# SSTDV-Project/python-fluid-simulation

Measured on AMD Instinct MI355X. Metric: PressureCGSolver3D CG throughput (cells x iterations / s), higher is better.
Workload: dtype f32; 1 GPU; PressureCGSolver3D 256x256x256 synthetic pool scene, fp32 state; cells_per_gpu=16777216, decomposition=single domain, transport=single, step=one CG iteration (apply + 2 dots + x/r/d updates)

## Files before the change

python-fluid-simulation_amd/csrc/mfs_pcg_apply.h:

```cpp
#pragma once
#include "mfs_common.h"
#include "mfs_cg_core.h"

#define MFS_LDS_BARRIER() asm volatile("s_waitcnt lgkmcnt(0)\n\ts_barrier" ::: "memory")

#ifndef MFS_MARCH_MIN_WAVES
#define MFS_MARCH_MIN_WAVES 3
#endif

namespace mfs {

constexpr int kApplyBlock = 256;
constexpr int kXcds = 8;

template <typename T, int VEC>
__device__ __forceinline__ void stencil_vec(T* __restrict__ out_ptr, vec_t<T, VEC> vc, vec_t<T, VEC> vxp,
                                            vec_t<T, VEC> vxm, vec_t<T, VEC> vyp, vec_t<T, VEC> vym,
                                            vec_t<T, VEC> dg, vec_t<T, VEC> cxp, vec_t<T, VEC> cxm,
                                            vec_t<T, VEC> cyp, vec_t<T, VEC> cym, vec_t<T, VEC> czm, double zl,
                                            double zr, double czr, bool first, bool last, bool active, double& acc,
                                            vec_t<T, VEC> czm2) {
  vec_t<T, VEC> o;
#ifdef MFS_APPLY_NATIVE_MATH
  typedef T C;
#else
  typedef double C;
#endif
#pragma unroll
  for (int j = 0; j < VEC; ++j) {
    const C zm = j == 0 ? (C)zl : (C)vc[j == 0 ? 0 : j - 1];
    const C zp = j == VEC - 1 ? (C)zr : (C)vc[j == VEC - 1 ? j : j + 1];
    const C czp = j == VEC - 1 ? (C)czr : (C)czm[j == VEC - 1 ? j : j + 1];
    C val = 0;
    val -= (C)cxp[j] * (C)vxp[j];
    val -= (C)cxm[j] * (C)vxm[j];
    val -= (C)cyp[j] * (C)vyp[j];
    val -= (C)cym[j] * (C)vym[j];
    val -= czp * zp;
    val -= (C)czm2[j] * zm;
    val += (C)dg[j] * (C)vc[j];
    o[j] = (T)val;
    const bool bnd = (first && j == 0) || (last && j == VEC - 1);
    if (active && !bnd) acc += (double)vc[j] * (double)o[j];
  }
  if (!active) return;
  if (!first && !last) {
    vstore<T, VEC>(out_ptr, o);
  } else {
#pragma unroll
    for (int j = 0; j < VEC; ++j) {
      const bool bnd = (first && j == 0) || (last && j == VEC - 1);
      if (!bnd) out_ptr[j] = o[j];
    }
  }
}

struct ApplyArgs {
  int Nx, Ny, Nz, xb, xe, xchunk, xb2, xe2;
  const int* items = nullptr;
  const int* runrem = nullptr;
  const int* count = nullptr;
};

template <typename T, int VEC>
__global__ void __launch_bounds__(kApplyBlock)
k_pcg_apply_direct(const T* __restrict__ v, T* __restrict__ out, const T* __restrict__ diag,
                   const T* __restrict__ cx, const T* __restrict__ cy, const T* __restrict__ cz, ApplyArgs a,
                   double* __restrict__ partial, const double* __restrict__ done_flag) {
  if (done_flag && *done_flag != 0.0) return;
  const int nzv = a.Nz / VEC;
  const int64_t ipp = (int64_t)(a.Ny - 2) * nzv;
  const int n1 = a.xe - a.xb;
  const int np = n1 + (a.xe2 - a.xb2);
  const int nch = min((int)gridDim.x, kXcds);
  const int xcd = blockIdx.x % nch, slot = blockIdx.x / nch;
  const int nblk = (gridDim.x - xcd + nch - 1) / nch;
  const int p0 = (int)((int64_t)np * xcd / nch), p1 = (int)((int64_t)np * (xcd + 1) / nch);
  const int64_t end = (int64_t)p1 * ipp, stride = (int64_t)nblk * kApplyBlock;
  const int64_t sx = (int64_t)a.Ny * a.Nz, sy = a.Nz;
  double acc = 0.0;
  for (int64_t it = (int64_t)p0 * ipp + (int64_t)slot * kApplyBlock + threadIdx.x; it < end; it += stride) {
    const int px = (int)(it / ipp);
    const int rem = (int)(it - (int64_t)px * ipp);
    const int yy = rem / nzv, zv = rem - (rem / nzv) * nzv;
    const int xx = px < n1 ? a.xb + px : a.xb2 + (px - n1);
    const int64_t base = (int64_t)xx * sx + (int64_t)(yy + 1) * sy + (int64_t)zv * VEC;
    const bool first = zv == 0, last = zv == nzv - 1;
    const auto vc = vload<T, VEC>(v + base);
    const double zl = first ? 0.0 : (double)v[base - 1];
    const double zr = last ? 0.0 : (double)v[base + VEC];
    const double czr = last ? 0.0 : (double)cz[base + VEC];
    stencil_vec<T, VEC>(out + base, vc, vload<T, VEC>(v + base + sx), vload<T, VEC>(v + base - sx),
                        vload<T, VEC>(v + base + sy), vload<T, VEC>(v + base - sy), vload<T, VEC>(diag + base),
                        vload<T, VEC>(cx + base + sx), vload<T, VEC>(cx + base), vload<T, VEC>(cy + base + sy),
                        vload<T, VEC>(cy + base), vload<T, VEC>(cz + base), zl, zr, czr, first, last, true, acc,
                        vload<T, VEC>(cz + base));
  }
  const double tot = block_sum<kApplyBlock>(acc);
  if (threadIdx.x == 0) partial[blockIdx.x] = tot;
}


template <typename T, int VEC>
struct CoefVec {
  vec_t<T, VEC> dg, cxm, cxp, cym, cyp, czm, czm2;
  unsigned char cls;
};

template <typename T, int VEC, bool COMP, int NT, bool LOAD_CXM = true, bool ASYM = false>
__device__ __forceinline__ CoefVec<T, VEC> coef_load(const T* __restrict__ diag, const T* __restrict__ cx,
                                                     const T* __restrict__ cy, const T* __restrict__ cz,
                                                     int64_t b, int64_t sx, int Nz, unsigned char cls,
                                                     const T* __restrict__ cz2 = nullptr) {
  CoefVec<T, VEC> c;
  c.cls = cls;
  if (COMP) {
    const T f = cls == kClsRegular ? (T)1 : (T)0, d = cls == kClsRegular ? (T)6 : (T)0;
#pragma unroll
    for (int j = 0; j < VEC; ++j) { c.dg[j] = d; c.cxm[j] = f; c.cxp[j] = f; c.cym[j] = f; c.cyp[j] = f; c.czm[j] = f; c.czm2[j] = f; }
    if (cls == kClsMixed) {
      c.dg = (NT & 1) ? vload_nt<T, VEC>(diag + b) : vload<T, VEC>(diag + b);
      if (LOAD_CXM) c.cxm = vload<T, VEC>(cx + b);
      c.cxp = (NT & 2) ? vload_nt<T, VEC>(cx + b + sx) : vload<T, VEC>(cx + b + sx);
      c.cym = (NT & 4) ? vload_nt<T, VEC>(cy + b) : vload<T, VEC>(cy + b);
      c.cyp = (NT & 4) ? vload_nt<T, VEC>(cy + b + Nz) : vload<T, VEC>(cy + b + Nz);
      c.czm = (NT & 1) ? vload_nt<T, VEC>(cz + b) : vload<T, VEC>(cz + b);
      if (ASYM) c.czm2 = (NT & 1) ? vload_nt<T, VEC>(cz2 + b) : vload<T, VEC>(cz2 + b);
    }
    if (!ASYM) c.czm2 = c.czm;
    return c;
  }
  c.dg = (NT & 1) ? vload_nt<T, VEC>(diag + b) : vload<T, VEC>(diag + b);
  c.cxm = c.dg;
  c.cxp = (NT & 2) ? vload_nt<T, VEC>(cx + b + sx) : vload<T, VEC>(cx + b + sx);
  c.cym = (NT & 4) ? vload_nt<T, VEC>(cy + b) : vload<T, VEC>(cy + b);
  c.cyp = (NT & 4) ? vload_nt<T, VEC>(cy + b + Nz) : vload<T, VEC>(cy + b + Nz);
  c.czm = (NT & 1) ? vload_nt<T, VEC>(cz + b) : vload<T, VEC>(cz + b);
  if (ASYM) c.czm2 = (NT & 1) ? vload_nt<T, VEC>(cz2 + b) : vload<T, VEC>(cz2 + b);
  else c.czm2 = c.czm;
  return c;
}

template <typename T, int VEC>
__global__ void __launch_bounds__(256)
k_pcg_classify(const T* __restrict__ diag, const T* __restrict__ cx, const T* __restrict__ cy,
               const T* __restrict__ cz, int Nx, int Ny, int Nz, unsigned char* __restrict__ cls,
               const T* __restrict__ cz2) {
  const int nzv = Nz / VEC;
  const int64_t nvec = (int64_t)Nx * Ny * nzv;
  const int64_t iv = (int64_t)blockIdx.x * blockDim.x + threadIdx.x;
  if (iv >= nvec) return;
  const int zv = (int)(iv % nzv), y = (int)((iv / nzv) % Ny), x = (int)(iv / ((int64_t)nzv * Ny));
  const int64_t sx = (int64_t)Ny * Nz, b = iv * VEC;
  bool all_zero = true, all_reg = true;
  if (x > 0 && x < Nx - 1 && y > 0 && y < Ny - 1) {
#pragma unroll
    for (int j = 0; j < VEC; ++j) {
      const int z = zv * VEC + j;
      if (z == 0 || z == Nz - 1) continue;
      const int64_t c = b + j;
      const T k[7] = {diag[c], cx[c], cx[c + sx], cy[c], cy[c + Nz], cz2 ? cz2[c] : cz[c], cz[c + 1]};
      bool z0 = true, r1 = k[0] == (T)6;
#pragma unroll
      for (int q = 0; q < 7; ++q) { z0 = z0 && k[q] == (T)0; if (q) r1 = r1 && k[q] == (T)1; }
      if (cz2 && j == 0) { z0 = z0 && cz[c] == (T)0; r1 = r1 && cz[c] == (T)1; }
      all_zero = all_zero && z0;
      all_reg = all_reg && r1;
    }
  }
  cls[iv] = all_zero ? kClsZero : (all_reg ? kClsRegular : kClsMixed);
}

template <typename T, int VEC>
struct RawVec { vec_t<T, VEC> a, b; };

template <typename T, int VEC, bool FUSE>
struct VSrc {
  const T* __restrict__ v;
  const T* __restrict__ r;
  const T* __restrict__ d_old;
  double beta;
  __device__ __forceinline__ RawVec<T, VEC> raw(int64_t off) const {
    RawVec<T, VEC> w;
    if (!FUSE) { w.a = vload<T, VEC>(v + off); w.b = w.a; }
    else { w.a = vload<T, VEC>(r + off); w.b = vload<T, VEC>(d_old + off); }
    return w;
  }
  __device__ __forceinline__ vec_t<T, VEC> fin(const RawVec<T, VEC>& w) const {
    if (!FUSE) return w.a;
    vec_t<T, VEC> o;
#pragma unroll
    for (int j = 0; j < VEC; ++j) o[j] = (T)((double)w.a[j] + beta * (double)w.b[j]);
    return o;
  }
  __device__ __forceinline__ vec_t<T, VEC> ld(int64_t off) const { return fin(raw(off)); }
};

struct BookArgs {
  double* scal;
  double* hist;
  int64_t hist_cap;
  const double* part_rr;
  int npart, par;
};

template <typename T, int VEC, bool LDS, int NT, bool COMP, bool FUSE, int PD, bool ASYM = false, bool XDEF = false,
          bool BOOK = false, bool LMASK = false>
__global__ void __launch_bounds__(kApplyBlock, MFS_MARCH_MIN_WAVES)
k_pcg_apply_march(const T* __restrict__ v, T* __restrict__ out, const T* __restrict__ diag,
                  const T* __restrict__ cx, const T* __restrict__ cy, const T* __restrict__ cz,
                  const unsigned char* __restrict__ cls, ApplyArgs a, double* __restrict__ partial,
                  const double* __restrict__ done_flag, const T* __restrict__ fr, const T* __restrict__ fd_old,
                  T* __restrict__ fd_new, const double* __restrict__ beta_ptr, const T* __restrict__ cz2,
                  T* __restrict__ xdef = nullptr, const double* __restrict__ alpha_ptr = nullptr, BookArgs bk = BookArgs{}) {
  static_assert(!XDEF || FUSE, "the deferred x update rides on the fused direction update");
  static_assert(!LMASK || (COMP && FUSE && PD == 1), "lane-level masking: compressed, fused, prefetch depth 1");
  static_assert(!BOOK || FUSE, "closing the previous iteration rides on the fused direction update");
  static_assert(kApplyBlock == kBlock, "block_total_of is written for kBlock threads");
  double alpha_x = (XDEF && !BOOK) ? *alpha_ptr : 0.0;
  static_assert(!FUSE || LDS, "the fused direction update is implemented on the LDS march");
  double bk_dn = 0.0, bk_delta = 0.0, bk_dq = 0.0, bk_tol2 = 0.0, bk_acc = 0.0;
  bool book_pending = BOOK;
  double beta_v = 0.0;
  if (BOOK) {
    bk_dn = bk.scal[S_DONE]; bk_delta = bk.scal[S_RING + bk.par]; bk_dq = bk.scal[S_DQ]; bk_tol2 = bk.scal[S_TOL2];
    for (int i = threadIdx.x; i < bk.npart; i += kBlock) bk_acc += bk.part_rr[i];
  } else {
    if (done_flag && *done_flag != 0.0) return;
    if (FUSE) beta_v = *beta_ptr;
  }
  VSrc<T, VEC, FUSE> src{v, fr, fd_old, beta_v};
  extern __shared__ __align__(16) unsigned char smem_raw[];
  T* const smem = reinterpret_cast<T*>(smem_raw);
  const int Nz = a.Nz;
  const int nzv = Nz / VEC;
  const int ipp = (a.Ny - 2) * nzv;
  const int tiles = (ipp + kApplyBlock - 1) / kApplyBlock;
  const int n1 = a.xe - a.xb;
  const int np = n1 + (a.xe2 - a.xb2);
  const bool sparse = a.items != nullptr;
  const int64_t total = sparse ? (int64_t)*a.count : (int64_t)tiles * np;

  const int G = gridDim.x;
  const int nch = min(G, kXcds);
  const int xcd = blockIdx.x % nch, slot = blockIdx.x / nch;
  const int per = G / nch, extra = G - per * nch;
  const int seg = xcd * per + min(xcd, extra) + slot;
  const int64_t s0 = total * seg / G, s1 = total * (seg + 1) / G;
  const int64_t sx = (int64_t)a.Ny * Nz;
  const int tid = threadIdx.x, lane = tid & 63;
  const int tile_elems = kApplyBlock * VEC;
  const int buf_elems = tile_elems + 2 * Nz;
  double acc = 0.0;

  auto close_previous = [&]() -> bool {
    book_pending = false;
    __shared__ double s_rr;
    const double t = block_sum<kBlock>(bk_acc);
    if (threadIdx.x == 0) s_rr = t;
    __syncthreads();
    const double rr = s_rr;
    const bool stop = bk_dn != 0.0 || cg_health(bk_dq, rr) != 0 || rr < bk_tol2;
    if (bk_dn == 0.0 && blockIdx.x == 0 && threadIdx.x == 0) cg_book(bk.scal, bk.hist, bk.hist_cap, bk.par, bk_dq, rr);
    src.beta = rr / bk_delta;
    if (XDEF) alpha_x = bk_delta / bk_dq;
    return stop;
  };

  for (int64_t i = s0; i < s1;) {
    const int64_t it_ = sparse ? (int64_t)a.items[i] : i;
    const int tile = (int)(it_ / np);
    const int pl = (int)(it_ - (int64_t)tile * np);
    const int x0 = pl < n1 ? a.xb + pl : a.xb2 + (pl - n1);
    int len = (int)min((int64_t)((pl < n1 ? a.xe : a.xe2) - x0), s1 - i);
    if (sparse) len = min(len, a.runrem[i]);
    if (a.xchunk > 0) len = min(len, a.xchunk);
    const int x1 = x0 + len;
    i += len;
    const int item_raw = tile * kApplyBlock + tid;
    const bool active = item_raw < ipp;
    const int item = active ? item_raw : ipp - 1;
    const int yy = item / nzv, zv = item - yy * nzv;
    const bool first = zv == 0, last = zv == nzv - 1;
    const int64_t m = (int64_t)(yy + 1) * Nz + (int64_t)zv * VEC;
    const int64_t m0 = (int64_t)Nz + (int64_t)tile * tile_elems;
    const int tile_len = min(tile_elems, ipp * VEC - tile * tile_elems);

    int64_t base = (int64_t)x0 * sx + m;
    const RawVec<T, VEC> wm = src.raw(base - sx), wc = src.raw(base), wp = src.raw(base + sx);
    constexpr bool MASK = LMASK;
    const bool mask_on = MASK && sparse;
    unsigned char cls_n = kClsMixed, cls_c = kClsMixed, cls_n2 = kClsMixed;
    if (COMP) {
      cls_c = cls[base / VEC];
      cls_n = cls[(base + (x0 + 1 < x1 ? sx : 0)) / VEC];
      if (MASK) cls_n2 = cls[((int64_t)min(x0 + 2, x1) * sx + m) / VEC];
    }
    RawVec<T, VEC> wh = {};
    const bool h0 = LDS && tid < 2 * nzv;
    if (h0) wh = src.raw((int64_t)x0 * sx + (tid < nzv ? m0 - Nz + tid * VEC : m0 + tile_len + (tid - nzv) * VEC));
    if (BOOK && book_pending) {
      if (close_previous()) return;
    }
    vec_t<T, VEC> vm = src.fin(wm), vc = src.fin(wc), vp = src.fin(wp);
    CoefVec<T, VEC> cc = coef_load<T, VEC, COMP, NT, true, ASYM>(diag, cx, cy, cz, base, sx, Nz, cls_c, cz2);
    if (!COMP) cc.cxm = vload<T, VEC>(cx + base);

    if (LDS) {
      T* b0 = smem;
      if (active) vstore<T, VEC>(b0 + Nz + tid * VEC, vc);
      if (h0) vstore<T, VEC>(b0 + (tid < nzv ? tid * VEC : Nz + tile_len + (tid - nzv) * VEC), src.fin(wh));
      for (int s = tid + kApplyBlock; s < 2 * nzv; s += kApplyBlock) {
        const bool lo = s < nzv;
        const int j = lo ? s : s - nzv;
        vstore<T, VEC>(b0 + (lo ? j * VEC : Nz + tile_len + j * VEC),
                       src.ld((int64_t)x0 * sx + (lo ? m0 - Nz + j * VEC : m0 + tile_len + j * VEC)));
      }
      MFS_LDS_BARRIER();
    }
    const bool hact = LDS && tid < 2 * nzv;
    const bool hlow = tid < nzv;
    const int64_t hg = hlow ? m0 - Nz + (int64_t)tid * VEC : m0 + tile_len + (int64_t)(tid - nzv) * VEC;
    const int hl = hlow ? tid * VEC : Nz + tile_len + (tid - nzv) * VEC;
    RawVec<T, VEC> Q[PD > 1 ? PD - 1 : 1], H[PD];
#pragma unroll
    for (int k = 0; k < PD - 1; ++k) Q[k] = src.raw((int64_t)min(x0 + 2 + k, x1) * sx + m);
#pragma unroll
    for (int k = 0; k < PD; ++k) {
      H[k] = RawVec<T, VEC>{};
      if (hact) H[k] = src.raw((int64_t)min(x0 + 1 + k, x1) * sx + hg);
    }

    for (int x = x0; x < x1; ++x) {
      const bool more = x + 1 < x1;
      const int cur = (x - x0) & 1;
      const int64_t nb = base + sx;
      const int64_t nn = more ? nb : base;
      const int64_t n2 = more ? nb + sx : nb;
      const bool dead_c = mask_on && cc.cls == kClsDead;
      RawVec<T, VEC> qn = {};
      if (!(mask_on && cls_n2 == kClsDead)) qn = src.raw((int64_t)min(x + 1 + PD, x1) * sx + m);
      vec_t<T, VEC> xo = {}, dxo = {};
      if (XDEF && !dead_c) { xo = vload_nt<T, VEC>(xdef + base); dxo = vload<T, VEC>(fd_old + base); }
      CoefVec<T, VEC> cn = coef_load<T, VEC, COMP, NT, false, ASYM>(diag, cx, cy, cz, nn, sx, Nz, more ? cls_n : cc.cls, cz2);
      cn.cxm = cc.cxp;
      unsigned char cls_nn = kClsMixed;
      if (COMP) cls_nn = MASK ? cls[((int64_t)min(x + 3, x1) * sx + m) / VEC] : cls[n2 / VEC];
      RawVec<T, VEC> hn = {};
      if (hact) hn = src.raw((int64_t)min(x + 1 + PD, x1) * sx + hg);
      vec_t<T, VEC> vym, vyp;
      double zl, zr;
      if (LDS) {
        const T* bc = smem + cur * buf_elems;
        vym = vload<T, VEC>(bc + tid * VEC);
        vyp = vload<T, VEC>(bc + 2 * Nz + tid * VEC);
        zl = (double)bc[Nz + tid * VEC - 1];
        zr = (double)bc[Nz + tid * VEC + VEC];
      } else {
        vym = vload<T, VEC>(v + base - Nz);
        vyp = vload<T, VEC>(v + base + Nz);
        const T l = __shfl_up(vc[VEC - 1], 1, 64), r = __shfl_down(vc[0], 1, 64);
        zl = (double)((lane == 0 && !first) ? v[base - 1] : l);
        zr = (double)((lane == 63 && !last) ? v[base + VEC] : r);
      }
      const T czs = __shfl_down(cc.czm[0], 1, 64);
      const double czr = (double)((lane == 63 && !last) ? cz[base + VEC] : czs);
      stencil_vec<T, VEC>(out + base, vc, vp, vm, vyp, vym, cc.dg, cc.cxp, cc.cxm, cc.cyp, cc.cym, cc.czm, zl, zr, czr,
                          first, last, active && !dead_c, acc, cc.czm2);
      if (FUSE && active && !dead_c) vstore<T, VEC>(fd_new + base, vc);
      if (XDEF && active && !dead_c) {
#pragma unroll
        for (int j = 0; j < VEC; ++j) xo[j] = (T)((double)xo[j] + alpha_x * (double)dxo[j]);
        vstore_nt<T, VEC>(xdef + base, xo);
      }
      if (more) {
        if (LDS) {
          T* bn = smem + (cur ^ 1) * buf_elems;
          if (active) vstore<T, VEC>(bn + Nz + tid * VEC, vp);
          if (hact) vstore<T, VEC>(bn + hl, src.fin(H[0]));
          for (int s = tid + kApplyBlock; s < 2 * nzv; s += kApplyBlock) {
            const bool lo = s < nzv;
            const int j = lo ? s : s - nzv;
            vstore<T, VEC>(bn + (lo ? j * VEC : Nz + tile_len + j * VEC),
                           src.ld((int64_t)(x + 1) * sx + (lo ? m0 - Nz + j * VEC : m0 + tile_len + j * VEC)));
          }
          MFS_LDS_BARRIER();
        }
        vm = vc; vc = vp; vp = src.fin(PD == 1 ? qn : Q[0]); cc = cn;
        if (MASK) { cls_n = cls_n2; cls_n2 = cls_nn; } else cls_n = cls_nn;
#pragma unroll
        for (int k = 0; k + 1 < PD - 1; ++k) Q[k] = Q[k + 1];
        if (PD > 1) Q[PD - 2] = qn;
#pragma unroll
        for (int k = 0; k + 1 < PD; ++k) H[k] = H[k + 1];
        H[PD - 1] = hn;
        base = nb;
      }
    }
    if (LDS) MFS_LDS_BARRIER();
  }
  if (BOOK && book_pending) {
    if (close_previous()) return;
  }
  const double tot = block_sum<kApplyBlock>(acc);
  if (threadIdx.x == 0) partial[blockIdx.x] = tot;
}

}
```

Baseline: 191,900 Mcells/s.

## Reuse streamed direction values for deferred x update and reorder marching loads/stores

The deferred x += alpha*d_old update now takes d_old from the raw direction value already streamed for the stencil (the .b half of the fused source), so the separate fd_old reload is gone. The x loads are prefetched two planes ahead to match the stencil's read-ahead. The stencil is split into compute and store, and empty asm register constraints force the next plane's loads to be waited on before the output stores are issued. The z-edge coefficient is also prefetched one plane ahead. This cuts global reads and reorders the memory queue, but raises register pressure and restricts the deferred-x path to prefetch depth 1.

Result: faster. 194,700 Mcells/s (median of 6 runs) (+1.4%).

```diff
diff --git a/python-fluid-simulation_amd/csrc/mfs_pcg_apply.h b/python-fluid-simulation_amd/csrc/mfs_pcg_apply.h
--- a/python-fluid-simulation_amd/csrc/mfs_pcg_apply.h
+++ b/python-fluid-simulation_amd/csrc/mfs_pcg_apply.h
@@ -14,12 +14,12 @@
 constexpr int kXcds = 8;
 
 template <typename T, int VEC>
-__device__ __forceinline__ void stencil_vec(T* __restrict__ out_ptr, vec_t<T, VEC> vc, vec_t<T, VEC> vxp,
-                                            vec_t<T, VEC> vxm, vec_t<T, VEC> vyp, vec_t<T, VEC> vym,
-                                            vec_t<T, VEC> dg, vec_t<T, VEC> cxp, vec_t<T, VEC> cxm,
-                                            vec_t<T, VEC> cyp, vec_t<T, VEC> cym, vec_t<T, VEC> czm, double zl,
-                                            double zr, double czr, bool first, bool last, bool active, double& acc,
-                                            vec_t<T, VEC> czm2) {
+__device__ __forceinline__ vec_t<T, VEC> stencil_calc(vec_t<T, VEC> vc, vec_t<T, VEC> vxp,
+                                                      vec_t<T, VEC> vxm, vec_t<T, VEC> vyp, vec_t<T, VEC> vym,
+                                                      vec_t<T, VEC> dg, vec_t<T, VEC> cxp, vec_t<T, VEC> cxm,
+                                                      vec_t<T, VEC> cyp, vec_t<T, VEC> cym, vec_t<T, VEC> czm, double zl,
+                                                      double zr, double czr, bool first, bool last, bool active, double& acc,
+                                                      vec_t<T, VEC> czm2) {
   vec_t<T, VEC> o;
 #ifdef MFS_APPLY_NATIVE_MATH
   typedef T C;
@@ -43,6 +43,11 @@
     const bool bnd = (first && j == 0) || (last && j == VEC - 1);
     if (active && !bnd) acc += (double)vc[j] * (double)o[j];
   }
+  return o;
+}
+
+template <typename T, int VEC>
+__device__ __forceinline__ void stencil_put(T* __restrict__ out_ptr, vec_t<T, VEC> o, bool first, bool last, bool active) {
   if (!active) return;
   if (!first && !last) {
     vstore<T, VEC>(out_ptr, o);
@@ -54,6 +59,20 @@
     }
   }
 }
+
+template <typename T, int VEC>
+__device__ __forceinline__ void stencil_vec(T* __restrict__ out_ptr, vec_t<T, VEC> vc, vec_t<T, VEC> vxp,
+                                            vec_t<T, VEC> vxm, vec_t<T, VEC> vyp, vec_t<T, VEC> vym,
+                                            vec_t<T, VEC> dg, vec_t<T, VEC> cxp, vec_t<T, VEC> cxm,
+                                            vec_t<T, VEC> cyp, vec_t<T, VEC> cym, vec_t<T, VEC> czm, double zl,
+                                            double zr, double czr, bool first, bool last, bool active, double& acc,
+                                            vec_t<T, VEC> czm2) {
+  stencil_put<T, VEC>(out_ptr, stencil_calc<T, VEC>(vc, vxp, vxm, vyp, vym, dg, cxp, cxm, cyp, cym, czm, zl, zr, czr, first,
+                                                    last, active, acc, czm2), first, last, active);
+}
+
+template <typename S>
+__device__ __forceinline__ void vm_arrived(S s) { asm volatile("" ::"v"(s)); }
 
 struct ApplyArgs {
   int Nx, Ny, Nz, xb, xe, xchunk, xb2, xe2;
@@ -213,7 +232,7 @@
                   const double* __restrict__ done_flag, const T* __restrict__ fr, const T* __restrict__ fd_old,
                   T* __restrict__ fd_new, const double* __restrict__ beta_ptr, const T* __restrict__ cz2,
                   T* __restrict__ xdef = nullptr, const double* __restrict__ alpha_ptr = nullptr, BookArgs bk = BookArgs{}) {
-  static_assert(!XDEF || FUSE, "the deferred x update rides on the fused direction update");
+  static_assert(!XDEF || (FUSE && PD == 1), "the deferred x update rides on the fused direction update, prefetch depth 1");
   static_assert(!LMASK || (COMP && FUSE && PD == 1), "lane-level masking: compressed, fused, prefetch depth 1");
   static_assert(!BOOK || FUSE, "closing the previous iteration rides on the fused direction update");
   static_assert(kApplyBlock == kBlock, "block_total_of is written for kBlock threads");
@@ -299,9 +318,17 @@
     RawVec<T, VEC> wh = {};
     const bool h0 = LDS && tid < 2 * nzv;
     if (h0) wh = src.raw((int64_t)x0 * sx + (tid < nzv ? m0 - Nz + tid * VEC : m0 + tile_len + (tid - nzv) * VEC));
+    const bool zedge = lane == 63 && !last;
+    T cze = (T)0;
+    if (zedge) cze = cz[base + VEC];
     if (BOOK && book_pending) {
       if (close_previous()) return;
     }
+    const bool xu0 = XDEF && active && !(mask_on && cls_c == kClsDead);
+    const bool xu1 = XDEF && active && x0 + 1 < x1 && !(mask_on && cls_n == kClsDead);
+    vec_t<T, VEC> xa = {}, xb = {};
+    if (xu0) xa = vload_nt<T, VEC>(xdef + base);
+    if (xu1) xb = vload_nt<T, VEC>(xdef + base + sx);
     vec_t<T, VEC> vm = src.fin(wm), vc = src.fin(wc), vp = src.fin(wp);
     CoefVec<T, VEC> cc = coef_load<T, VEC, COMP, NT, true, ASYM>(diag, cx, cy, cz, base, sx, Nz, cls_c, cz2);
     if (!COMP) cc.cxm = vload<T, VEC>(cx + base);
@@ -318,6 +345,16 @@
       }
       MFS_LDS_BARRIER();
     }
+    if (xu0) {
+#pragma unroll
+      for (int j = 0; j < VEC; ++j) xa[j] = (T)((double)xa[j] + alpha_x * (double)wc.b[j]);
+      vstore_nt<T, VEC>(xdef + base, xa);
+    }
+    if (xu1) {
+#pragma unroll
+      for (int j = 0; j < VEC; ++j) xb[j] = (T)((double)xb[j] + alpha_x * (double)wp.b[j]);
+      vstore_nt<T, VEC>(xdef + base + sx, xb);
+    }
     const bool hact = LDS && tid < 2 * nzv;
     const bool hlow = tid < nzv;
     const int64_t hg = hlow ? m0 - Nz + (int64_t)tid * VEC : m0 + tile_len + (int64_t)(tid - nzv) * VEC;
@@ -340,14 +377,17 @@
       const bool dead_c = mask_on && cc.cls == kClsDead;
       RawVec<T, VEC> qn = {};
       if (!(mask_on && cls_n2 == kClsDead)) qn = src.raw((int64_t)min(x + 1 + PD, x1) * sx + m);
-      vec_t<T, VEC> xo = {}, dxo = {};
-      if (XDEF && !dead_c) { xo = vload_nt<T, VEC>(xdef + base); dxo = vload<T, VEC>(fd_old + base); }
+      const bool xu = XDEF && active && x + 2 < x1 && !(mask_on && cls_n2 == kClsDead);
+      vec_t<T, VEC> xq = {};
+      if (xu) xq = vload_nt<T, VEC>(xdef + base + 2 * sx);
       CoefVec<T, VEC> cn = coef_load<T, VEC, COMP, NT, false, ASYM>(diag, cx, cy, cz, nn, sx, Nz, more ? cls_n : cc.cls, cz2);
       cn.cxm = cc.cxp;
       unsigned char cls_nn = kClsMixed;
       if (COMP) cls_nn = MASK ? cls[((int64_t)min(x + 3, x1) * sx + m) / VEC] : cls[n2 / VEC];
       RawVec<T, VEC> hn = {};
       if (hact) hn = src.raw((int64_t)min(x + 1 + PD, x1) * sx + hg);
+      T czn = (T)0;
+      if (zedge) czn = cz[nn + VEC];
       vec_t<T, VEC> vym, vyp;
       double zl, zr;
       if (LDS) {
@@ -364,15 +404,11 @@
         zr = (double)((lane == 63 && !last) ? v[base + VEC] : r);
       }
       const T czs = __shfl_down(cc.czm[0], 1, 64);
-      const double czr = (double)((lane == 63 && !last) ? cz[base + VEC] : czs);
-      stencil_vec<T, VEC>(out + base, vc, vp, vm, vyp, vym, cc.dg, cc.cxp, cc.cxm, cc.cyp, cc.cym, cc.czm, zl, zr, czr,
-                          first, last, active && !dead_c, acc, cc.czm2);
-      if (FUSE && active && !dead_c) vstore<T, VEC>(fd_new + base, vc);
-      if (XDEF && active && !dead_c) {
-#pragma unroll
-        for (int j = 0; j < VEC; ++j) xo[j] = (T)((double)xo[j] + alpha_x * (double)dxo[j]);
-        vstore_nt<T, VEC>(xdef + base, xo);
-      }
+      const double czr = (double)(zedge ? cze : czs);
+      const vec_t<T, VEC> o = stencil_calc<T, VEC>(vc, vp, vm, vyp, vym, cc.dg, cc.cxp, cc.cxm, cc.cyp, cc.cym, cc.czm, zl, zr,
+                                                   czr, first, last, active && !dead_c, acc, cc.czm2);
+#pragma unroll
+      for (int j = 0; j < VEC; ++j) vm_arrived(o[j]);
       if (more) {
         if (LDS) {
           T* bn = smem + (cur ^ 1) * buf_elems;
@@ -386,7 +422,19 @@
           }
           MFS_LDS_BARRIER();
         }
-        vm = vc; vc = vp; vp = src.fin(PD == 1 ? qn : Q[0]); cc = cn;
+      }
+      vm_arrived(qn.a[0]); vm_arrived(qn.b[0]); vm_arrived(xq[0]);
+      vm_arrived(cn.dg[0]); vm_arrived(cn.cxp[0]); vm_arrived(cn.cym[0]); vm_arrived(cn.cyp[0]); vm_arrived(cn.czm[0]);
+      vm_arrived(cn.czm2[0]); vm_arrived((int)cls_nn); vm_arrived(hn.a[0]); vm_arrived(hn.b[0]); vm_arrived(czn);
+      stencil_put<T, VEC>(out + base, o, first, last, active && !dead_c);
+      if (FUSE && active && !dead_c) vstore<T, VEC>(fd_new + base, vc);
+      if (more) {
+        if (xu) {
+#pragma unroll
+          for (int j = 0; j < VEC; ++j) xq[j] = (T)((double)xq[j] + alpha_x * (double)qn.b[j]);
+          vstore_nt<T, VEC>(xdef + base + 2 * sx, xq);
+        }
+        vm = vc; vc = vp; vp = src.fin(PD == 1 ? qn : Q[0]); cc = cn; cze = czn;
         if (MASK) { cls_n = cls_n2; cls_n2 = cls_nn; } else cls_n = cls_nn;
 #pragma unroll
         for (int k = 0; k + 1 < PD - 1; ++k) Q[k] = Q[k + 1];
```
